# PKU-EPIC/PartManip

Hardware: AMD Instinct MI355X
Metric: PPO env-steps/sec (whole node), 4096 envs x 1024-pt clouds (higher is better)
Workload: dtype f32

## Files before the change

include/partmanip_hip.h:

```cpp
#ifndef PARTMANIP_HIP_H
#define PARTMANIP_HIP_H

#include <stddef.h>
#include <stdint.h>

#ifdef __cplusplus
extern "C" {
#endif

#define PM_OK 0
#define PM_EINVAL (-1)
#define PM_EWORKSPACE (-2)
#define PM_EALIGN (-3)
#define PM_EUNSUPPORTED (-4)

#define PM_ACT_NONE 0
#define PM_ACT_TANH 1
#define PM_ACT_RELU 2
#define PM_ACT_LRELU 3
#define PM_ACT_ELU 4
#define PM_ACT_SELU 5
#define PM_ACT_SIGMOID 6
#define PM_ACT_MAX 6

// ... 11 lines not shown
int pm_adv_normalize_f32(float* x, long n, float eps, void* workspace, size_t workspace_bytes, void* stream);

int pm_gather_rows_f32(const float* src, const int64_t* idx, float* dst, long n_rows, long row_elems,
                       long src_ld, long dst_ld, void* stream);

int pm_linear_fwd_f32(const float* X, long ldx, const float* W, long ldw, const float* b, float* Y, long ldy,
                      int M, int N, int K, int act, void* stream);
int pm_linear_bwd_data_f32(const float* dY, long lddy, const float* W, long ldw, const float* H, long ldh,
                           float* dX, long lddx, int M, int N, int K, int act, void* stream);
size_t pm_linear_bwd_weight_workspace_bytes(int M, int N, int K);
int pm_linear_bwd_weight_f32(const float* dY, long lddy, const float* X, long ldx, float* dW, long lddw,
                             float* db, int M, int N, int K, void* workspace, size_t workspace_bytes,
                             void* stream);

int pm_mlp_fwd_f32(const float* X, long ldx, int M, int n_layers, const int* dims, const float* const* W, const float* const* b,
                   int act, float* const* H, void* stream);
size_t pm_mlp_bwd_workspace_bytes(int M, int n_layers, const int* dims);
int pm_mlp_bwd_f32(const float* X, long ldx, int M, int n_layers, const int* dims, const float* const* W, const float* const* H,
                   int act, const float* dY, float* const* dW, float* const* db, float* dX, void* workspace,
                   size_t workspace_bytes, void* stream);

#define PM_LINEAR_GROUP_MAX 8
typedef struct pm_linear_fwd_desc {
    const float* X; long ldx; const float* W; long ldw; const float* b; float* Y; long ldy; int M, N, K, act;
} pm_linear_fwd_desc;
typedef struct pm_linear_bwd_data_desc {
    const float* dY; long lddy; const float* W; long ldw; const float* H; long ldh; float* dX; long lddx; int M, N, K, act;
} pm_linear_bwd_data_desc;
typedef struct pm_linear_bwd_weight_desc {
    const float* dY; long lddy; const float* X; long ldx; float* dW; long lddw; float* db; long slab_stride; int M, N, K;
    int dy_cols, x_cols;
    int pad_;
} pm_linear_bwd_weight_desc;
int pm_linear_fwd_group_f32(int n, const pm_linear_fwd_desc* d, void* stream);
int pm_linear_bwd_data_group_f32(int n, const pm_linear_bwd_data_desc* d, void* stream);
int pm_linear_bwd_weight_group_f32(int n, const pm_linear_bwd_weight_desc* d, int splits, void* stream);
#define PM_LINEAR_PATH_SKINNY 0
#define PM_LINEAR_PATH_REG 1
#define PM_LINEAR_PATH_DMA 2
typedef struct pm_linear_variant {
    int path;
    int tm, tn;
    int lay;
    int stages;
    int vec;
    int big;
    int grid;
    int n;
    int vecC[PM_LINEAR_GROUP_MAX];
    int splits[PM_LINEAR_GROUP_MAX];
    int kchunk[PM_LINEAR_GROUP_MAX];
} pm_linear_variant;
int pm_linear_fwd_variant_f32(const float* X, long ldx, const float* W, long ldw, const float* b, const float* Y, long ldy,
                              int M, int N, int K, int act, pm_linear_variant* out);
int pm_linear_bwd_data_variant_f32(const float* dY, long lddy, const float* W, long ldw, const float* H, long ldh,
                                   const float* dX, long lddx, int M, int N, int K, int act, pm_linear_variant* out);
int pm_linear_bwd_weight_variant_f32(const float* dY, long lddy, const float* X, long ldx, const float* dW, long lddw,
                                     const float* db, int M, int N, int K, const void* workspace, pm_linear_variant* out);
int pm_linear_fwd_group_variant_f32(int n, const pm_linear_fwd_desc* d, pm_linear_variant* out);
int pm_linear_bwd_data_group_variant_f32(int n, const pm_linear_bwd_data_desc* d, pm_linear_variant* out);
int pm_linear_bwd_weight_group_variant_f32(int n, const pm_linear_bwd_weight_desc* d, int splits, pm_linear_variant* out);
size_t pm_linear_chain_workspace_bytes(int M);
int pm_linear_fwd_chain_f32(int n, const pm_linear_fwd_desc* d, void* workspace, size_t workspace_bytes, void* stream);
int pm_linear_bwd_data_chain_f32(int n, const pm_linear_bwd_data_desc* d, void* workspace, size_t workspace_bytes, void* stream);

size_t pm_pointnet_packed_elems(void);
int pm_pointnet_pack_weights_f32(const float* W2, const float* W3, float* packed, void* stream);
int pm_pointnet_enc_fwd_f32(const float* x, long ldx, int B, int P, int C, int sub_mean, const float* W1,
                            const float* b1, const float* b2, const float* b3, const float* packed,
                            int max_mean, float* feat, long ldf, int32_t* argmax,
                            float* h2_save ,
                            int act ,
                            void* stream);
size_t pm_pointnet_packed_screen_bytes(void);
int pm_pointnet_pack_weights_screen(const float* W3, const float* b3, void* packed, void* stream);
int pm_pointnet_enc_fwd_screen_f32(const float* x, long ldx, int B, int P, int C, int sub_mean, const float* W1,
                                   const float* b1, const float* b2, const float* b3, const float* packed,
                                   const void* packed_screen, int max_mean, float* feat, long ldf, int32_t* argmax,
                                   float* h2_save, unsigned long long* counters, void* stream);
int pm_pointnet_enc_fwd_screen_sched_f32(const float* x, long ldx, int B, int P, int C, int sub_mean, const float* W1,
                                         const float* b1, const float* b2, const float* b3, const float* packed,
                                         const void* packed_screen, int max_mean, float* feat, long ldf, int32_t* argmax,
                                         float* h2_save, unsigned long long* counters, int schedule, void* stream);
size_t pm_pointnet_packed_bf3_bytes(void);
int pm_pointnet_pack_weights_bf3(const float* W2, const float* W3, void* packed, void* stream);
int pm_pointnet_enc_fwd_bf3(const float* x, long ldx, int B, int P, int C, int sub_mean, const float* W1,
                            const float* b1, const float* b2, const float* b3, const void* packed, int max_mean,
                            float* feat, long ldf, int32_t* argmax, float* h2_save ,
                            void* stream);
size_t pm_pointnet_packed_bf6_bytes(void);
int pm_pointnet_pack_weights_bf6(const float* W2, const float* W3, void* packed, void* stream);
int pm_pointnet_enc_fwd_bf6(const float* x, long ldx, int B, int P, int C, int sub_mean, const float* W1,
                            const float* b1, const float* b2, const float* b3, const void* packed, int max_mean,
                            float* feat, long ldf, int32_t* argmax, float* h2_save ,
                            void* stream);
size_t pm_pointnet_enc_bwd_workspace_bytes(int B, int P, int C);
int pm_pointnet_enc_bwd_f32(const float* x, long ldx, int B, int P, int C, int sub_mean, const float* W1,
                            const float* b1, const float* b2, const float* W3, const float* packed,
                            int max_mean, const float* dfeat, long ldf, const int32_t* argmax, float* dW1,
                            float* db1, float* dW2, float* db2, float* dW3, float* db3,
                            const float* h2_saved ,
                            int act , void* workspace, size_t workspace_bytes, void* stream);
int pm_pointnet_enc_bwd_w4_f32(const float* x, long ldx, int B, int P, int C, int sub_mean, const float* W1,
                               const float* b1, const float* b2, const float* W3, const float* packed,
                               int max_mean, const float* dfeat, long ldf, const int32_t* argmax, float* dW1,
                               float* db1, float* dW2, float* db2, float* dW3, float* db3, const float* h2_saved,
                               int act, void* workspace, size_t workspace_bytes, void* stream);
size_t pm_pointnet_packed_bwd_bf6_bytes(void);
int pm_pointnet_pack_weights_bwd_bf6(const float* W2, void* packed, void* stream);
int pm_pointnet_enc_bwd_bf6(const float* x, long ldx, int B, int P, int C, int sub_mean, const float* W1,
                            const float* b1, const float* b2, const float* W3, const float* packed,
                            const void* packed_w2_bf6, int max_mean, const float* dfeat, long ldf, const int32_t* argmax,
                            float* dW1, float* db1, float* dW2, float* db2, float* dW3, float* db3, const float* h2_saved,
                            void* workspace, size_t workspace_bytes, void* stream);

int pm_ppo_actor_loss_fwd_bwd_f32(const float* mu, long ldmu, const float* log_std, const float* actions,
                                  long lda, const float* old_logp, const float* adv, const float* old_mu,
                                  long ldom, const float* old_sigma, long ldos, int B, int A, float max_action,
                                  int act_tanh, float eps_clip, float desired_kl, const double* adv_moments,
                                  double adv_count, float* scal_out, float* dmu, long lddmu, float* dlog_std,
                                  void* workspace, size_t workspace_bytes, void* stream);
size_t pm_ppo_actor_loss_workspace_bytes(int B);
int pm_ppo_actor_head_supported(const float* H, long ldh, const float* W, long ldw, int A, int K, const float* dH, long lddh);
int pm_ppo_actor_head_f32(const float* H, long ldh, const float* W, long ldw, const float* bias, int K, int hidden_act,
                          const float* log_std, const float* actions, long lda, const float* old_logp, const float* adv,
                          const float* old_mu, long ldom, const float* old_sigma, long ldos, int B, int A, float max_action,
                          int act_tanh, float eps_clip, float desired_kl, const double* adv_moments, double adv_count,
                          float* scal_out, float* mu_out, long ldmu, float* dmu, long lddmu, float* dH, long lddh,
                          float* dlog_std, void* workspace, size_t workspace_bytes, unsigned int* counter, void* stream);
int pm_gaussian_logp_f32(const float* mu, long ldmu, const float* log_std, const float* actions, long lda,
                         int B, int A, float max_action, int act_tanh, float* logp, float* entropy,
                         void* stream);

int pm_value_loss_fwd_bwd_f32(const float* V, const float* returns, const float* old_values, int B,
                              int clipped, float eps_clip, const float* clip_mean_extern, float grad_scale,
                              float* scal_out, float* dV, long lddv, void* stream);

size_t pm_value_head_workspace_bytes(void);
int pm_value_head_supported(const float* H, long ldh, const float* W, int K, const float* dH, long lddh);
int pm_value_head_f32(const float* H, long ldh, const float* W, const float* bias, int K, int hidden_act, const float* returns,
                      const float* old_values, int B, int clipped, float eps_clip, const float* clip_mean_extern,
                      float grad_scale, float* scal_out, float* V_out, float* dV, long lddv, float* dH, long lddh,
                      void* workspace, size_t workspace_bytes, unsigned int* counter, void* stream);

int pm_mse_tanh_loss_fwd_bwd_f32(const float* stu_mu, long lds, const float* tea_mu, long ldt, int B, int A,
                                 float max_action, int act_tanh, float grad_scale, float* scal_out,
                                 float* dstu_mu, long ldd, void* stream);
int pm_action_activation_f32(const float* mu, float* out, long n, float max_action, int act_tanh, void* stream);
int pm_gaussian_logp_bwd_f32(const float* mu, long ldmu, const float* log_std, const float* actions, long lda, int B, int A,
                             float max_action, int act_tanh, const float* dlogp, const float* dent, float* dmu, long lddm,
                             float* dlog_std, void* stream);
int pm_action_activation_bwd_f32(const float* out, const float* dout, float* dmu, long n, float max_action, int act_tanh,
                                 void* stream);

size_t pm_clip_adam_workspace_bytes(long n);
typedef struct pm_clip_adam_desc {
    float* params; float* grads; float* exp_avg; float* exp_avg_sq; long n, n_clip; const float* extra; long extra_stride;
    long n_sum; int n_extra; float max_norm; double lr, b1, b2, eps; int32_t* state; const float* skip_flag;
    float* gnorm_out; void* workspace;
    float* stats_acc; const float* stats_scal; int stats_which;
    float grad_scale; float dp_kl_desired; float* dp_scal;
} pm_clip_adam_desc;
int pm_clip_adam_group_f32(int n, const pm_clip_adam_desc* d, void* stream);
int pm_grad_slab_sum_f32(float* grads, const float* extra, long extra_stride, long n_sum, int n_extra, void* stream);
int pm_clip_adam_step_f32(float* params, const float* grads, float* exp_avg, float* exp_avg_sq, long n,
                          long n_clip, float max_norm, double lr, double b1, double b2, double eps,
// ... 323 lines not shown
```

partmanip_amd/_lib.py:

```python
import ctypes as C
import os

import torch

HERE = os.path.dirname(os.path.abspath(__file__))
LIB_PATH = os.environ.get("PARTMANIP_HIP_LIB") or os.path.join(HERE, "lib", "libpartmanip_hip.so")

P, I, L, F, D, Z = C.c_void_p, C.c_int, C.c_long, C.c_float, C.c_double, C.c_size_t

SIGNATURES = {
    "pm_version": (I, []),
    "pm_gae_scan_f32": (I, [P, P, P, P, P, P, P, I, I, F, F, I, F, P]),
    "pm_moments_workspace_bytes": (Z, [L]),
    "pm_moments_f64": (I, [P, L, P, P, Z, P]),
    "pm_normalize_apply_f32": (I, [P, L, P, D, F, P]),
    "pm_gather_rows_f32": (I, [P, P, P, L, L, L, L, P]),
    "pm_linear_fwd_f32": (I, [P, L, P, L, P, P, L, I, I, I, I, P]),
    "pm_linear_bwd_data_f32": (I, [P, L, P, L, P, L, P, L, I, I, I, I, P]),
    "pm_linear_bwd_weight_workspace_bytes": (Z, [I, I, I]),
    "pm_linear_bwd_weight_f32": (I, [P, L, P, L, P, L, P, I, I, I, P, Z, P]),
    "pm_linear_fwd_group_f32": (I, [I, P, P]),
    "pm_linear_bwd_data_group_f32": (I, [I, P, P]),
    "pm_linear_chain_workspace_bytes": (C.c_size_t, [I]),
    "pm_linear_fwd_chain_f32": (I, [I, P, P, C.c_size_t, P]),
    "pm_linear_bwd_data_chain_f32": (I, [I, P, P, C.c_size_t, P]),
    "pm_linear_bwd_weight_group_f32": (I, [I, P, I, P]),
    "pm_linear_fwd_variant_f32": (I, [P, L, P, L, P, P, L, I, I, I, I, P]),
    "pm_linear_bwd_data_variant_f32": (I, [P, L, P, L, P, L, P, L, I, I, I, I, P]),
    "pm_linear_bwd_weight_variant_f32": (I, [P, L, P, L, P, L, P, I, I, I, P, P]),
    "pm_linear_fwd_group_variant_f32": (I, [I, P, P]),
    "pm_linear_bwd_data_group_variant_f32": (I, [I, P, P]),
    "pm_linear_bwd_weight_group_variant_f32": (I, [I, P, I, P]),
    "pm_clip_adam_group_f32": (I, [I, P, P]),
    "pm_grad_slab_sum_f32": (I, [P, P, L, L, I, P]),
    "pm_pointnet_packed_elems": (Z, []),
    "pm_pointnet_pack_weights_f32": (I, [P, P, P, P]),
    "pm_pointnet_enc_fwd_f32": (I, [P, L, I, I, I, I, P, P, P, P, P, I, P, L, P, P, I, P]),
    "pm_pointnet_packed_screen_bytes": (Z, []),
    "pm_pointnet_pack_weights_screen": (I, [P, P, P, P]),
    "pm_pointnet_enc_fwd_screen_f32": (I, [P, L, I, I, I, I, P, P, P, P, P, P, I, P, L, P, P, P, P]),
    "pm_pointnet_enc_fwd_screen_sched_f32": (I, [P, L, I, I, I, I, P, P, P, P, P, P, I, P, L, P, P, P, I, P]),
    "pm_pointnet_packed_bf3_bytes": (Z, []),
    "pm_pointnet_pack_weights_bf3": (I, [P, P, P, P]),
    "pm_pointnet_enc_fwd_bf3": (I, [P, L, I, I, I, I, P, P, P, P, P, I, P, L, P, P, P]),
    "pm_pointnet_packed_bf6_bytes": (Z, []),
    "pm_pointnet_pack_weights_bf6": (I, [P, P, P, P]),
    "pm_pointnet_enc_fwd_bf6": (I, [P, L, I, I, I, I, P, P, P, P, P, I, P, L, P, P, P]),
    "pm_pointnet_enc_bwd_workspace_bytes": (Z, [I, I, I]),
    "pm_pointnet_enc_bwd_f32": (I, [P, L, I, I, I, I, P, P, P, P, P, I, P, L, P, P, P, P, P, P, P, P, I, P, Z, P]),
    "pm_pointnet_enc_bwd_w4_f32": (I, [P, L, I, I, I, I, P, P, P, P, P, I, P, L, P, P, P, P, P, P, P, P, I, P, Z, P]),
    "pm_pointnet_packed_bwd_bf6_bytes": (Z, []),
    "pm_pointnet_pack_weights_bwd_bf6": (I, [P, P, P]),
    "pm_pointnet_enc_bwd_bf6": (I, [P, L, I, I, I, I, P, P, P, P, P, P, I, P, L, P, P, P, P, P, P, P, P, P, Z, P]),
    "pm_ppo_actor_loss_fwd_bwd_f32": (I, [P, L, P, P, L, P, P, P, L, P, L, I, I, F, I, F, F, P, D, P, P, L, P, P, Z, P]),
    "pm_ppo_actor_loss_workspace_bytes": (Z, [I]),
    "pm_ppo_actor_head_supported": (I, [P, L, P, L, I, I, P, L]),
    "pm_ppo_actor_head_f32": (I, [P, L, P, L, P, I, I, P, P, L, P, P, P, L, P, L, I, I, F, I, F, F, P, D, P, P, L, P, L, P, L, P, P, Z, P, P]),
    "pm_gaussian_logp_f32": (I, [P, L, P, P, L, I, I, F, I, P, P, P]),
    "pm_gaussian_logp_bwd_f32": (I, [P, L, P, P, L, I, I, F, I, P, P, P, L, P, P]),
    "pm_action_activation_bwd_f32": (I, [P, P, P, L, F, I, P]),
    "pm_value_loss_fwd_bwd_f32": (I, [P, P, P, I, I, F, P, F, P, P, L, P]),
    "pm_value_head_workspace_bytes": (Z, []),
    "pm_value_head_supported": (I, [P, L, P, I, P, L]),
    "pm_value_head_f32": (I, [P, L, P, P, I, I, P, P, I, I, F, P, F, P, P, P, L, P, L, P, Z, P, P]),
    "pm_mse_tanh_loss_fwd_bwd_f32": (I, [P, L, P, L, I, I, F, I, F, P, P, L, P]),
    "pm_action_activation_f32": (I, [P, P, L, F, I, P]),
    "pm_clip_adam_workspace_bytes": (Z, [L]),
    "pm_clip_adam_step_f32": (I, [P, P, P, P, L, L, F, D, D, D, D, P, P, P, P, Z, P]),
    "pm_ppo_accumulate_stats_f32": (I, [P, P, I, P]),
    "pm_fps_workspace_bytes": (Z, [I, I]),
    "pm_fps_f32": (I, [P, I, I, I, I, P, P, Z, P]),
    "pm_ball_query_f32": (I, [P, P, I, I, I, F, I, P, P]),
    "pm_group_points_f32": (I, [P, P, I, I, I, I, I, P, P]),
    "pm_group_points_bwd_f32": (I, [P, P, I, I, I, I, I, P, P]),
    "pm_group_concat_f32": (I, [P, P, P, P, I, I, I, I, I, I, P, P]),
    "pm_group_concat_bwd_f32": (I, [P, P, I, I, I, I, I, I, P, P]),
    "pm_maxpool_rows_f32": (I, [P, L, I, I, P, L, P, P]),
    "pm_maxpool_rows_bwd_f32": (I, [P, L, P, L, I, I, P, P, P]),
    "pm_depth_backproject_f32": (I, [P, I, I, I, I, P, F, F, F, F, P, P, P, P]),
    "pm_depth_compact_f32": (I, [P, I, I, P, P, P]),
    "pm_depth_cloud_f32": (I, [P, I, I, I, I, P, F, F, F, F, P, P, I, P, P, P, P]),
    "pm_cloud_gather_labeled_f32": (I, [P, P, I, I, P, I, P, L, I, F, P, L, P]),
    "pm_fps_varlen_f32": (I, [P, I, I, I, I, P, I, P, P, Z, P]),
    "pm_fps_varlen_workspace_bytes": (Z, [I, I]),
    "pm_tsdf_select_f32": (I, [P, I, I, F, F, P, P, P]),
    "pm_gaussian_sample_f32": (I, [P, L, P, P, I, I, F, I, P, P, P, P]),
    "pm_rms_update_workspace_bytes": (Z, [I]),
    "pm_rms_update_f32": (I, [P, L, I, I, I, P, P, P, P, Z, P]),
    "pm_rms_normalize_f32": (I, [P, L, I, I, P, P, P, L, P]),
    "pm_rms_moments_f64": (I, [P, L, I, I, P, P, Z, P]),
    "pm_rms_apply_moments_f32": (I, [P, L, I, I, P, P, P, P]),
    "pm_tsdf_sparse_gather_f32": (I, [P, P, P, I, I, I, P, P]),
    "pm_im2col3d_f32": (I, [P, I, I, I, I, I, I, I, I, L, L, L, L, L, P, I, P]),
    "pm_conv3d_c1_supported": (I, [I, I]),
    "pm_conv3d_c1_wgrad_workspace_bytes": (Z, [I]),
    "pm_conv3d_c1_fwd_f32": (I, [P, I, I, I, I, I, I, I, L, L, L, L, P, P, I, I, P, L, P, P]),
    "pm_conv3d_c1_wgrad_f32": (I, [P, L, P, I, I, I, I, I, I, I, L, L, L, L, I, P, L, P, P, P, Z, P]),
    "pm_col2im3d_f32": (I, [P, I, I, I, I, I, I, I, I, L, L, L, L, L, P, I, P, I, P]),
    "pm_tsdf_integrate_f32": (I, [P, P, P, I, I, L, L, F, F, P, P]),
    "pm_mesh_tsdf_query_f32": (I, [P, P, P, P, P, P, P, I, I, I, I, I, F, F, F, F, F, P, I, P, L, I, P]),
    "pm_mesh_tsdf_query_groups_f32": (I, [P, P, P, P, P, P, I, I, P, I, P, I, P, P, I, I, I, I, I, F, F, F, F, F, P, I, P, L, I, P]),
    "pm_mesh_sdf_bake_workspace_bytes": (Z, [I]),
    "pm_mesh_sdf_bake_f32": (I, [P, I, I, I, I, F, F, F, F, F, I, P, P, Z, P]),
    "pm_mesh_pc_query_f32": (I, [P, P, I, P, P, I, I, P, L, I, P, L, P]),
    "pm_mesh_pc_query_labeled_f32": (I, [P, P, I, P, P, I, I, P, L, I, P, L, P, P]),
    "pm_mesh_depth_render_f32": (I, [P, P, I, P, I, P, P, I, I, P, I, F, F, F, F, I, I, F, F, P, L, P]),
    "pm_mesh_frame_workspace_bytes": (Z, [I, I, I, I]),
    "pm_mesh_frame_render_f32": (I, [P, P, I, P, I, P, P, I, I, P, I, F, F, F, F, I, I, F, F, P, I, P, F, F, I, I, I, P, L, P, L, P, L, P, Z,
                                     P]),
    "pm_mesh_depth_render_groups_f32": (I, [P, P, I, P, I, I, P, I, P, I, P, P, I, I, P, I, F, F, F, F, I, I, F, F, P, L, P]),
    "pm_mesh_frame_render_groups_f32": (I, [P, P, I, P, I, I, P, I, P, I, P, P, I, I, P, I, F, F, F, F, I, I, F, F, P, I, P, F, F, I, I, I,
                                            P, L, P, L, P, L, P, Z, P]),
    "pm_body_pose_gather_f32": (I, [P, L, P, I, I, P, I, P, P, P]),
    "pm_grasp_cube_post_f32": (I, [P, P, P, I, I, I, I, I, I, I, P, P, P, P, P, F, P, P, P, I, P, L, P, L, P, P, P, P, L, P, P, P]),
    "pm_franka_control_f32": (I, [P, L, I, P, P, I, I, I, I, I, P, P, P, F, I, P, P, P, I, I, I, P, P, P, P, P, P, I, P]),
    "pm_franka_control_mobile_f32": (I, [P, L, I, P, P, I, I, I, I, I, P, P, P, F, I, I, P, P, P, P, I, I, I, P, P, P, P, P, P, I, P]),
    "pm_open_drawer_post_f32": (I, [P, L, P, L, P, I, I, I, I, I, I, I, P, P, P, I, P, P, P, P, P, P, F, P, P, I, P, L, P, P, P, P, P, L, P, P, P,
                                    P, P, P]),
    "pm_open_drawer_reset_f32": (I, [P, P, P, I, I, I, I, I, P, P, I, P, F, F, P, P, P, P, L, P, P, P, P]),
    "pm_articulation_step_f32": (I, [P, P, P, P, P, P, P, P, P, P, F, P, L, P, L, P, L, P, P, L, L, P, L, I, I, I, P, P, P]),
    "pm_articulation_objects_step_f32": (I, [P, P, I, I, I, I, I, P, P, P, P, P, P, P, P, P, P, P, P, L, P, P, P, L, P, L, P, P, P, P, F, I, P]),
    "pm_free_body_step_f32": (I, [P, L, P, P, P, I, I, P, P, P, P, P, F, F, F, F, I, P]),
    "pm_voxel_grid0_f32": (I, [P, L, I, I, I, I, P, P, P, P]),
    "pm_voxel_nbr27_i32": (I, [P, L, P, I, P, I, P]),
# ... 129 lines not shown
```

partmanip_amd/build.py:

```python
import os
import subprocess
import sys

HERE = os.path.dirname(os.path.abspath(__file__))
CSRC = os.path.join(HERE, "csrc")
LIBDIR = os.path.join(HERE, "lib")
LIB = os.path.join(LIBDIR, "libpartmanip_hip.so")
SOURCES = ["gae.hip", "losses.hip", "adam.hip", "gemm_f32.hip", "gemm2_f32.hip", "pointnet_enc.hip", "pointnet_enc_bf3.hip", "pointnet_enc_bf6.hip", "pointops.hip", "sa_fused.hip", "sa_groupall.hip", "conv3d.hip", "sparse_voxel.hip", "bn_pool2d.hip", "mesh_tsdf.hip", "mesh_bake.hip", "mesh_pc.hip", "mesh_depth.hip", "mesh_frame.hip", "body_pose.hip", "task_grasp_cube.hip", "task_open_drawer.hip", "articulation.hip", "articulation_objects.hip", "free_body.hip"]
FLAGS = ["-O3", "-std=c++17", "--offload-arch=gfx950", "-fPIC", "-ffp-contract=off", "-Wall",
         "-Wno-unused-function"]


def _newer(a, b):
    return (not os.path.exists(b)) or os.path.getmtime(a) > os.path.getmtime(b)


def build(force=False, verbose=False):
    hipcc = os.environ.get("HIPCC", "/opt/rocm/bin/hipcc")
    os.makedirs(LIBDIR, exist_ok=True)
    objdir = os.path.join(LIBDIR, "obj")
    os.makedirs(objdir, exist_ok=True)
    hdrs = [os.path.join(CSRC, "common.h"), os.path.join(CSRC, "mfma_f32.h"), os.path.join(CSRC, "gemm2.h"), os.path.join(CSRC, "skinny.h"), os.path.join(CSRC, "pointnet_enc_bwd_bf6.h"), os.path.join(CSRC, "pointnet_enc_screen.h"), os.path.join(CSRC, "task_common.h"), os.path.join(CSRC, "articulation_common.h"), os.path.join(CSRC, "mesh_raster.h"),
            os.path.join(HERE, "..", "include", "partmanip_hip.h")]
    objs, rebuilt = [], False
    procs = []
    for src in SOURCES:
        s = os.path.join(CSRC, src)
        o = os.path.join(objdir, src.replace(".hip", ".o"))
        objs.append(o)
        if force or _newer(s, o) or any(_newer(h, o) for h in hdrs):
            cmd = [hipcc, "-x", "hip", "-c", s, "-o", o] + FLAGS
            if verbose:
                print(" ".join(cmd))
            procs.append((src, subprocess.Popen(cmd, stdout=subprocess.PIPE, stderr=subprocess.STDOUT)))
            rebuilt = True
    for src, p in procs:
        out, _ = p.communicate()
        if p.returncode != 0:
            sys.stderr.write(out.decode())
            raise RuntimeError(f"hipcc failed on {src}")
        if verbose and out:
            print(out.decode())
    if rebuilt or not os.path.exists(LIB):
        cmd = [hipcc, "-shared", "-fPIC", "--offload-arch=gfx950", "-o", LIB] + objs
        subprocess.run(cmd, check=True)
    return LIB


if __name__ == "__main__":
    print(build(force="--force" in sys.argv, verbose=True))
```

partmanip_amd/csrc/pointnet_enc_screen.h:

```cpp
#pragma once

typedef _Float16 ps_f16x8 __attribute__((ext_vector_type(8)));

#define PS_LDP (PN_C2 + 8)
#define PS_CAP 256
#define PS_NW 8
#define PS_P3 (16 * 16 * 64 * 8)
#define PS_OFF_P3 0
#define PS_OFF_W3 (2 * PS_P3)
#define PS_OFF_EPS (PS_OFF_W3 + PN_C3 * PN_C2 * 4)
#define PS_OFF_INV (PS_OFF_EPS + PN_C3 * 4)
#define PS_PACKED_BYTES (PS_OFF_INV + PN_C3 * 4)
#ifndef PS_ABLATE
#define PS_ABLATE 0
#endif
#ifndef PS_SCHED_DEFAULT
#define PS_SCHED_DEFAULT 0
#endif

extern "C" size_t pm_pointnet_packed_screen_bytes(void) { return PS_PACKED_BYTES; }

__device__ __forceinline__ unsigned ps_cvt_pk(float a, float b) {
    unsigned r;
    asm("v_cvt_pk_f16_f32 %0, %1, %2" : "=v"(r) : "v"(a), "v"(b));
    return r;
}

__global__ __launch_bounds__(PN_C2) void ps_pack_kernel(const float* __restrict__ W3, const float* __restrict__ b3,
                                                         unsigned char* __restrict__ packed) {
    __shared__ double Ls[PN_C2], Rs[PN_C2], Ss[PN_C2];
    __shared__ float Ms[PN_C2];
    const int c = blockIdx.x, k = threadIdx.x;
    const float w = W3[c * PN_C2 + k];
    const float aw = fabsf(w);
    Ls[k] = (double)aw;
    Ms[k] = aw < INFINITY ? aw : 0.f;
    __syncthreads();
    for (int o = PN_C2 / 2; o > 0; o >>= 1) {
        if (k < o) {
            Ls[k] += Ls[k + o];
            Ms[k] = fmaxf(Ms[k], Ms[k + o]);
        }
        __syncthreads();
    }
    int ex = -200;
    if (Ms[0] > 0.f) frexpf(Ms[0], &ex);
    const int s = min(15 - ex, 126);
    const float ws = ldexpf(w, s);
    const _Float16 w16 = (_Float16)ws;
    const float wf = (float)w16, d = fabsf(ws - wf);
    Rs[k] = (double)(fabsf(wf) < 0x1p-14f ? fmaxf(fabsf(ws), d) : d);
    Ss[k] = (double)fabsf(wf);
    __syncthreads();
    for (int o = PN_C2 / 2; o > 0; o >>= 1) {
        if (k < o) {
            Rs[k] += Rs[k + o];
            Ss[k] += Ss[k + o];
        }
        __syncthreads();
    }
    const int nb = c >> 5, li = c & 31, step = k >> 4, lq = (k >> 3) & 1, e = k & 7;
    ((_Float16*)(packed + PS_OFF_P3))[(((nb * 16 + step) * 64) + lq * 32 + li) * 8 + e] = w16;
    ((float*)(packed + PS_OFF_W3))[c * PN_C2 + k] = w;
    if (k == 0) {
        const double ed = ((Rs[0] + 0x1p-12 * Ss[0]) * ldexp(1.0, -s) + 1024.0 * 0x1p-24 * (Ls[0] + fabs((double)b3[c]))) * (1.0 + 0x1p-10) + 0x1p-116;
        float ef = (float)ed;
        if ((double)ef < ed) ef = __uint_as_float(__float_as_uint(ef) + 1);
        ((float*)(packed + PS_OFF_EPS))[c] = ef;
        ((float*)(packed + PS_OFF_INV))[c] = ldexpf(1.f, -s);
    }
}

extern "C" int pm_pointnet_pack_weights_screen(const float* W3, const float* b3, void* packed, void* stream) {
    PM_REQUIRE(W3 && b3 && packed);
    if (((uintptr_t)packed & 15) != 0) return PM_EALIGN;
    hipLaunchKernelGGL(ps_pack_kernel, dim3(PN_C3), dim3(PN_C2), 0, pm_stream(stream), W3, b3, (unsigned char*)packed);
    PM_CHECK_LAUNCH();
    return PM_OK;
}

#define PS_MFMA(a, b, c) __builtin_amdgcn_mfma_f32_32x32x16_f16((a), (b), (c), 0, 0, 0)
__device__ __forceinline__ ps_f16x8 ps_h(const uint4& v) { return *(const ps_f16x8*)&v; }

__device__ __forceinline__ void ps_stream(const unsigned short* __restrict__ A, const uint4* __restrict__ B, f32x16 (&acc)[2][2]) {
    uint4 b0[2], b1[2], b2[2], b3[2], a0[2], a1[2];
#pragma unroll
    for (int nb = 0; nb < 2; ++nb) {
        b0[nb] = B[(size_t)(nb * 16 + 0) * 64];
        b1[nb] = B[(size_t)(nb * 16 + 1) * 64];
        b2[nb] = B[(size_t)(nb * 16 + 2) * 64];
    }
#pragma unroll
    for (int mb = 0; mb < 2; ++mb) a0[mb] = *(const uint4*)(A + mb * 32 * PS_LDP);
#define PS_STEP(S_, AC, AN, BC, BN, PFA, PFB)                                                  \
    {                                                                                          \
        if (PFA) {                                                                             \
            _Pragma("unroll") for (int mb = 0; mb < 2; ++mb)                                   \
                AN[mb] = *(const uint4*)(A + mb * 32 * PS_LDP + ((S_) + 1) * 16);              \
        }                                                                                      \
        if (PFB) {                                                                             \
            _Pragma("unroll") for (int nb = 0; nb < 2; ++nb)                                   \
                BN[nb] = B[(size_t)(nb * 16 + (S_) + 3) * 64];                                 \
        }                                                                                      \
// ... 89 lines not shown
    const float invr[2] = {invg[(wave * 2 + 0) * 32 + li0], invg[(wave * 2 + 1) * 32 + li0]};
    float w1r[4] = {0.f, 0.f, 0.f, 0.f}, b1r = 0.f;
    if constexpr (CT == 3 || CT == 4) layer1_row<CT>(W1, b1, w1r, b1r);

    const int ntiles = P / PN_TM;
    stage_points<PN_TM, NT>(xb, 0, C, sub_mean, cen, Xs);
    for (int tile = 0; tile < ntiles; ++tile) {
        int lane = lane0;
        asm volatile("" : "+v"(lane));
        const int li = lane & 31, lh = lane >> 5;
        PS_STAMP(0);
        __syncthreads();
        float xnext = 0.f;
        if (tile + 1 < ntiles) xnext = ps_point_load(xb, tile + 1, C, tid);
        if (!(PS_ABLATE & 1)) {
            if constexpr (CT == 3 || CT == 4) layer1_tile<CT, PN_TM, NT, true>(Xs, w1r, b1r, H);
            else layer1_tile<CT, PN_TM, NT, true>(Xs, W1, b1, C, H);
        }
        PS_STAMP(1);
        __syncthreads();
        {
            f32x16 acc2[2][1];
            zero_acc<2, 1>(acc2);
            if (PS_ABLATE & 2) {
#pragma unroll
                for (int mb = 0; mb < 2; ++mb)
#pragma unroll
                    for (int r = 0; r < 16; ++r)
                        acc2[mb][0][r] = H[(mb * 32 + (r & 3) + 8 * (r >> 2) + 4 * lh) * PN_LD1 + ((wave * 32 + li) & 127)];
            } else {
                layer2_mfma<2, 1>(H, P2v, wave, lane, acc2);
            }
            PS_STAMP(2);
            __syncthreads();
            PS_STAMP(3);
            const int col = wave * 32 + li;
            const float b2c = b2r;
            float ts = 0.f;
            const bool planes = !(PS_ABLATE & 8) || tile == 0;
            const bool odd = (lane & 1) != 0;
            unsigned* Hh2 = (unsigned*)(Hh + (odd ? PS_LDP : 0) + (col & ~1));
#pragma unroll
            for (int mb = 0; mb < 2; ++mb)
#pragma unroll
                for (int r = 0; r < 16; r += 2) {
                    const float z0 = acc2[mb][0][r] + b2c, z1 = acc2[mb][0][r + 1] + b2c;
                    f32x2 v2;
                    if (PS_ABLATE & 4) {
                        v2.x = z0;
                        v2.y = z1;
                    } else {
                        v2 = pm_tanh2(z0, z1);
                    }
                    const int row0 = mb * 32 + (r & 3) + 8 * (r >> 2) + 4 * lh;
                    H[row0 * PN_LD2 + col] = v2.x;
                    H[(row0 + 1) * PN_LD2 + col] = v2.y;
                    ts += v2.x;
                    ts += v2.y;
                    const float own = odd ? v2.y : v2.x, send = odd ? v2.x : v2.y;
                    const float recv = __int_as_float(__builtin_amdgcn_update_dpp(0, __float_as_int(send), 0xB1, 0xf, 0xf, false));
                    const float a = odd ? recv : own, c = odd ? own : recv;
                    if (planes) Hh2[row0 * (PS_LDP / 2)] = ps_cvt_pk(a, c);
                }
            ts += __shfl_xor(ts, 32, 64);
            csum += (double)ts;
            if (tile + 1 < ntiles) ps_point_store(xnext, sub_mean, cen, tid, Xs);
        }
        PS_STAMP(4);
        __syncthreads();
        PS_STAMP(5);

        const bool copy = h2_save && !(PS_ABLATE & 128), late = ps_late_wave<SCHED>(wave);
        float* h2dst = copy ? h2_save + ((long)b * P + (long)tile * PN_TM) * PN_C2 : nullptr;
        if (copy && late) ps_copy_h2<NT>(H, h2dst, tid);

        f32x16 acc[2][2];
        if (PS_ABLATE & 16) {
#pragma unroll
            for (int nb = 0; nb < 2; ++nb)
#pragma unroll
                for (int mb = 0; mb < 2; ++mb)
#pragma unroll
                    for (int r = 0; r < 16; ++r)
                        acc[mb][nb][r] = b3r[nb] + H[(mb * 32 + (r & 3) + 8 * (r >> 2) + 4 * lh) * PN_LD2 + ((wave * 64 + nb * 32 + li) & 255)];
        } else {
            zero_acc<2, 2>(acc);
            ps_stream(Hh + li * PS_LDP + lh * 8, S3 + (size_t)(wave * 2 * 16) * 64 + lane, acc);
        }
        PS_STAMP(6);

        unsigned msk[2];
        float tmax[2];
#if (PS_ABLATE & 32) && defined(__HIP_DEVICE_COMPILE__)
#pragma unroll
        for (int nb = 0; nb < 2; ++nb) {
#pragma unroll
            for (int mb = 0; mb < 2; ++mb) asm volatile("" ::"v"(acc[mb][nb]));
            msk[nb] = 0;
            tmax[nb] = 0.f;
        }
#else
#pragma unroll
        for (int nb = 0; nb < 2; ++nb) {
            float m = -INFINITY;
            const float iv = invr[nb], b3c = b3r[nb];
#pragma unroll
            for (int mb = 0; mb < 2; ++mb)
#pragma unroll
                for (int r = 0; r < 16; ++r) {
                    if (!(PS_ABLATE & 16)) acc[mb][nb][r] = fmaf(acc[mb][nb][r], iv, b3c);
                    m = fmaxf(m, acc[mb][nb][r]);
                }
            m = fmaxf(m, __shfl_xor(m, 32, 64));
            const float e = epsr[nb];
            const float vm = __shfl(vmax, nb * 32 + li, 64);
            const float thr = m - 2.f * e;
            unsigned k = 0;
#pragma unroll
            for (int mb = 0; mb < 2; ++mb)
#pragma unroll
                for (int r = 0; r < 16; ++r) {
                    const float z = acc[mb][nb][r];
                    const bool s = !(z < thr) && !(z + e <= vm);
                    k |= (s ? 1u : 0u) << (mb * 16 + r);
                }
            msk[nb] = k;
            tmax[nb] = m;
        }
#endif
        const int n = __popc(msk[0]) + __popc(msk[1]);
        int incl = n;
#pragma unroll
        for (int o = 1; o < 64; o <<= 1) {
            const int t = __shfl_up(incl, o, 64);
            if (lane >= o) incl += t;
        }
        const int total = __builtin_amdgcn_readlane(incl, 63);
        PS_STAMP(7);

        if (PS_ABLATE & 64) {
            vmax = fmaxf(vmax, lh ? tmax[1] : tmax[0]);
            if (counters && lane == 0) atomicAdd(counters + 0, (unsigned long long)total);
        } else if (total <= PS_CAP) {
            int off = incl - n;
#pragma unroll
            for (int nb = 0; nb < 2; ++nb) {
                unsigned m = msk[nb];
                while (m) {
                    const int bit = __ffs(m) - 1;
                    m &= m - 1;
                    const int row = (bit >> 4) * 32 + (bit & 3) + 8 * ((bit & 15) >> 2) + 4 * lh;
                    skey[wave][off++] = (row << 6) | (nb * 32 + li);
                }
            }
            __builtin_amdgcn_wave_barrier();
            const int j = lane & 7, g = lane >> 3;
            for (int e0 = 0; e0 < total; e0 += 8) {
                const int e = e0 + g;
                const int key = (e < total) ? skey[wave][e] : 0;
                const int row = key >> 6, cl = key & 63;
                const float* hp = H + row * PN_LD2 + 4 * j;
                const float* wp = W3r + (size_t)(wave * 64 + cl) * PN_C2 + 4 * j;
                float s = 0.f;
#pragma unroll
                for (int i = 0; i < 8; ++i) {
                    const float4 w = *(const float4*)(wp + 32 * i);
                    const float4 h = *(const float4*)(hp + 32 * i);
                    s = fmaf(w.x, h.x, s);
                    s = fmaf(w.y, h.y, s);
                    s = fmaf(w.z, h.z, s);
                    s = fmaf(w.w, h.w, s);
                }
                s += __shfl_xor(s, 4, 64);
                s += __shfl_xor(s, 2, 64);
                s += __shfl_xor(s, 1, 64);
                s += b3[wave * 64 + cl];
#pragma unroll
                for (int gg = 0; gg < 8; ++gg)
                    if (e0 + gg < total) {
                        const int kk = __builtin_amdgcn_readlane(key, gg * 8);
                        const float v = __int_as_float(__builtin_amdgcn_readlane(__float_as_int(s), gg * 8));
                        if ((kk & 63) == lane) {
                            const int p = tile * PN_TM + (kk >> 6);
                            if (!(fabsf(v) < INFINITY)) pois += v;
                            if (v > vmax || (v == vmax && p < imax)) {
                                vmax = v;
                                imax = p;
                            }
                        }
                    }
            }
            if (counters) {
                const unsigned long long h0 = __ballot(msk[0] != 0), h1 = __ballot(msk[1] != 0);
                if (lane == 0) {
                    atomicAdd(counters + 0, (unsigned long long)total);
                    atomicAdd(counters + 2, (unsigned long long)(__popc((unsigned)(h0 | (h0 >> 32))) + __popc((unsigned)(h1 | (h1 >> 32)))));
                }
            }
        } else {
#pragma unroll
            for (int nb = 0; nb < 2; ++nb) {
                const float b3c = b3r[nb];
#pragma unroll
                for (int r = 0; r < 16; ++r) acc[0][nb][r] = acc[1][nb][r] = b3c;
            }
            mfma_stream<2, 2, 32>(H + li * PN_LD2 + lh * 128, PN_LD2, P3v + (size_t)(wave * 2) * 32 * 64 + lane, acc);
#pragma unroll
            for (int nb = 0; nb < 2; ++nb) {
                float bv = -INFINITY, ps = 0.f;
                int bp = 0;
#pragma unroll
                for (int mb = 0; mb < 2; ++mb)
#pragma unroll
                    for (int r = 0; r < 16; ++r) {
                        const float v = acc[mb][nb][r];
                        if (!(fabsf(v) < INFINITY)) ps += v;
                        if (v > bv) {
                            bv = v;
                            bp = tile * PN_TM + mb * 32 + (r & 3) + 8 * (r >> 2) + 4 * lh;
                        }
                    }
                const float ov = __shfl_xor(bv, 32, 64), os = __shfl_xor(ps, 32, 64);
                const int op = __shfl_xor(bp, 32, 64);
                if (ov > bv || (ov == bv && op < bp)) {
                    bv = ov;
                    bp = op;
                }
                if (lh == nb) {
                    pois += ps + os;
                    if (bv > vmax || (bv == vmax && bp < imax)) {
                        vmax = bv;
                        imax = bp;
                    }
                }
            }
            if (counters && lane == 0) atomicAdd(counters + 1, 1ull);
        }
        PS_STAMP(8);
        if (copy && !late) ps_copy_h2<NT>(H, h2dst, tid);
        PS_STAMP(9);
    }
    if ((lane0 >> 5) == 0) cs[wave * 32 + lane0] = csum;
    __syncthreads();
    const int ch = tid;
    float v = vmax;
    if (pois != pois) v = pois;
    feat[(long)b * ldf + ch] = v;
    argmax[(long)b * PN_C3 + ch] = imax;
    if (max_mean) {
        const float* wr = W3r + (size_t)ch * PN_C2;
        double s = 0.0;
#pragma unroll 4
        for (int k = 0; k < PN_C2; k += 4) {
            const float4 w = *(const float4*)(wr + k);
            s = fma((double)w.x, cs[k], s);
            s = fma((double)w.y, cs[k + 1], s);
            s = fma((double)w.z, cs[k + 2], s);
            s = fma((double)w.w, cs[k + 3], s);
        }
        float mv = (float)(s / (double)P + (double)b3[ch]);
        if (pois != pois) mv = pois;
        feat[(long)b * ldf + PN_C3 + ch] = mv;
    }
}

extern "C" int pm_pointnet_enc_fwd_screen_sched_f32(const float* x, long ldx, int B, int P, int C, int sub_mean, const float* W1,
                                                    const float* b1, const float* b2, const float* b3, const float* packed,
                                                    const void* packed_screen, int max_mean, float* feat, long ldf,
                                                    int32_t* argmax, float* h2_save, unsigned long long* counters, int schedule,
                                                    void* stream) {
    PM_REQUIRE(x && W1 && b1 && b2 && b3 && packed && packed_screen && feat && argmax);
    PM_REQUIRE(schedule == 0 || schedule == 1);
    if (h2_save && ((uintptr_t)h2_save & 15) != 0) return PM_EALIGN;
    PM_REQUIRE(B > 0 && P > 0 && P % PN_TM == 0 && C >= 1 && C <= PN_MAXC && ldx >= (long)P * C);
    PM_REQUIRE(ldf >= PN_C3 * (max_mean ? 2 : 1));
    PM_REQUIRE(!sub_mean || C >= 3);
// ... 27 lines not shown
```

Before: 35970.

## Screen candidates in raw accumulator space with per-column thresholds and ballot compaction

```diff
diff --git a/include/partmanip_hip.h b/include/partmanip_hip.h
--- a/include/partmanip_hip.h
+++ b/include/partmanip_hip.h
@@ -117,6 +117,8 @@
                                          const float* b1, const float* b2, const float* b3, const float* packed,
                                          const void* packed_screen, int max_mean, float* feat, long ldf, int32_t* argmax,
                                          float* h2_save, unsigned long long* counters, int schedule, void* stream);
+int pm_pointnet_screen_select_thresholds(const float* mt, const float* eps, const float* b3, const float* inv, const float* vmax,
+                                         long n, float* T);
 size_t pm_pointnet_packed_bf3_bytes(void);
 int pm_pointnet_pack_weights_bf3(const float* W2, const float* W3, void* packed, void* stream);
 int pm_pointnet_enc_fwd_bf3(const float* x, long ldx, int B, int P, int C, int sub_mean, const float* W1,
diff --git a/partmanip_amd/_lib.py b/partmanip_amd/_lib.py
--- a/partmanip_amd/_lib.py
+++ b/partmanip_amd/_lib.py
@@ -40,6 +40,7 @@
     "pm_pointnet_pack_weights_screen": (I, [P, P, P, P]),
     "pm_pointnet_enc_fwd_screen_f32": (I, [P, L, I, I, I, I, P, P, P, P, P, P, I, P, L, P, P, P, P]),
     "pm_pointnet_enc_fwd_screen_sched_f32": (I, [P, L, I, I, I, I, P, P, P, P, P, P, I, P, L, P, P, P, I, P]),
+    "pm_pointnet_screen_select_thresholds": (I, [P, P, P, P, P, L, P]),
     "pm_pointnet_packed_bf3_bytes": (Z, []),
     "pm_pointnet_pack_weights_bf3": (I, [P, P, P, P]),
     "pm_pointnet_enc_fwd_bf3": (I, [P, L, I, I, I, I, P, P, P, P, P, I, P, L, P, P, P]),
diff --git a/partmanip_amd/build.py b/partmanip_amd/build.py
--- a/partmanip_amd/build.py
+++ b/partmanip_amd/build.py
@@ -20,7 +20,7 @@
     os.makedirs(LIBDIR, exist_ok=True)
     objdir = os.path.join(LIBDIR, "obj")
     os.makedirs(objdir, exist_ok=True)
-    hdrs = [os.path.join(CSRC, "common.h"), os.path.join(CSRC, "mfma_f32.h"), os.path.join(CSRC, "gemm2.h"), os.path.join(CSRC, "skinny.h"), os.path.join(CSRC, "pointnet_enc_bwd_bf6.h"), os.path.join(CSRC, "pointnet_enc_screen.h"), os.path.join(CSRC, "task_common.h"), os.path.join(CSRC, "articulation_common.h"), os.path.join(CSRC, "mesh_raster.h"),
+    hdrs = [os.path.join(CSRC, "common.h"), os.path.join(CSRC, "mfma_f32.h"), os.path.join(CSRC, "gemm2.h"), os.path.join(CSRC, "skinny.h"), os.path.join(CSRC, "pointnet_enc_bwd_bf6.h"), os.path.join(CSRC, "pointnet_enc_screen.h"), os.path.join(CSRC, "pointnet_enc_screen_select.h"), os.path.join(CSRC, "task_common.h"), os.path.join(CSRC, "articulation_common.h"), os.path.join(CSRC, "mesh_raster.h"),
             os.path.join(HERE, "..", "include", "partmanip_hip.h")]
     objs, rebuilt = [], False
     procs = []
diff --git a/partmanip_amd/csrc/pointnet_enc_screen.h b/partmanip_amd/csrc/pointnet_enc_screen.h
--- a/partmanip_amd/csrc/pointnet_enc_screen.h
+++ b/partmanip_amd/csrc/pointnet_enc_screen.h
@@ -1,4 +1,5 @@
 #pragma once
+#include "pointnet_enc_screen_select.h"
 
 typedef _Float16 ps_f16x8 __attribute__((ext_vector_type(8)));
 
@@ -19,6 +20,13 @@
 #endif
 
 extern "C" size_t pm_pointnet_packed_screen_bytes(void) { return PS_PACKED_BYTES; }
+
+extern "C" int pm_pointnet_screen_select_thresholds(const float* mt, const float* eps, const float* b3, const float* inv,
+                                                    const float* vmax, long n, float* T) {
+    PM_REQUIRE(mt && eps && b3 && inv && vmax && T && n >= 0);
+    for (long i = 0; i < n; ++i) T[i] = ps_select_threshold(mt[i], eps[i], b3[i], inv[i], vmax[i]);
+    return PM_OK;
+}
 
 __device__ __forceinline__ unsigned ps_cvt_pk(float a, float b) {
     unsigned r;
@@ -274,77 +282,74 @@
                 for (int mb = 0; mb < 2; ++mb)
 #pragma unroll
                     for (int r = 0; r < 16; ++r)
-                        acc[mb][nb][r] = b3r[nb] + H[(mb * 32 + (r & 3) + 8 * (r >> 2) + 4 * lh) * PN_LD2 + ((wave * 64 + nb * 32 + li) & 255)];
+                        acc[mb][nb][r] = ps_pow2_inverse(invr[nb]) * H[(mb * 32 + (r & 3) + 8 * (r >> 2) + 4 * lh) * PN_LD2 + ((wave * 64 + nb * 32 + li) & 255)];
         } else {
             zero_acc<2, 2>(acc);
             ps_stream(Hh + li * PS_LDP + lh * 8, S3 + (size_t)(wave * 2 * 16) * 64 + lane, acc);
         }
         PS_STAMP(6);
 
-        unsigned msk[2];
-        float tmax[2];
+        float T[2], tmax[2];
+        int total = 0;
+        unsigned long long hit[2] = {0ull, 0ull};
 #if (PS_ABLATE & 32) && defined(__HIP_DEVICE_COMPILE__)
 #pragma unroll
         for (int nb = 0; nb < 2; ++nb) {
 #pragma unroll
             for (int mb = 0; mb < 2; ++mb) asm volatile("" ::"v"(acc[mb][nb]));
-            msk[nb] = 0;
-            tmax[nb] = 0.f;
+            T[nb] = tmax[nb] = 0.f;
         }
 #else
 #pragma unroll
         for (int nb = 0; nb < 2; ++nb) {
             float m = -INFINITY;
-            const float iv = invr[nb], b3c = b3r[nb];
 #pragma unroll
             for (int mb = 0; mb < 2; ++mb)
 #pragma unroll
+                for (int r = 0; r < 16; ++r) m = fmaxf(m, acc[mb][nb][r]);
+            m = fmaxf(m, __shfl_xor(m, 32, 64));
+            const float mt = fmaf(m, invr[nb], b3r[nb]);
+            const float vm = __shfl(vmax, nb * 32 + li, 64);
+            T[nb] = ps_select_threshold(mt, epsr[nb], b3r[nb], invr[nb], vm);
+            tmax[nb] = mt;
+        }
+        int* const sk = skey[wave];
+#pragma unroll
+        for (int nb = 0; nb < 2; ++nb) {
+            const int kbase = (4 * lh) << 6 | (nb * 32 + li);
+#pragma unroll
+            for (int mb = 0; mb < 2; ++mb) {
+                bool sv[16];
+                unsigned long long mk[16];
+#pragma unroll
                 for (int r = 0; r < 16; ++r) {
-                    if (!(PS_ABLATE & 16)) acc[mb][nb][r] = fmaf(acc[mb][nb][r], iv, b3c);
-                    m = fmaxf(m, acc[mb][nb][r]);
-                }
-            m = fmaxf(m, __shfl_xor(m, 32, 64));
-            const float e = epsr[nb];
-            const float vm = __shfl(vmax, nb * 32 + li, 64);
-            const float thr = m - 2.f * e;
-            unsigned k = 0;
-#pragma unroll
-            for (int mb = 0; mb < 2; ++mb)
+                    sv[r] = !(acc[mb][nb][r] < T[nb]);
+                    mk[r] = __ballot(sv[r]);
+                }
+                __builtin_amdgcn_sched_barrier(0);
 #pragma unroll
                 for (int r = 0; r < 16; ++r) {
-                    const float z = acc[mb][nb][r];
-                    const bool s = !(z < thr) && !(z + e <= vm);
-                    k |= (s ? 1u : 0u) << (mb * 16 + r);
-                }
-            msk[nb] = k;
-            tmax[nb] = m;
+                    const bool s = sv[r];
+                    const unsigned long long mask = mk[r];
+                    if (__builtin_expect(mask != 0, 0)) {
+                        const int cnt = __popcll(mask);
+                        if (s && total + cnt <= PS_CAP) {
+                            const int pos = __builtin_amdgcn_mbcnt_hi((unsigned)(mask >> 32), __builtin_amdgcn_mbcnt_lo((unsigned)mask, total));
+                            sk[pos] = kbase + ((mb * 32 + (r & 3) + 8 * (r >> 2)) << 6);
+                        }
+                        total += cnt;
+                        hit[nb] |= mask;
+                    }
+                }
+            }
         }
 #endif
-        const int n = __popc(msk[0]) + __popc(msk[1]);
-        int incl = n;
-#pragma unroll
-        for (int o = 1; o < 64; o <<= 1) {
-            const int t = __shfl_up(incl, o, 64);
-            if (lane >= o) incl += t;
-        }
-        const int total = __builtin_amdgcn_readlane(incl, 63);
         PS_STAMP(7);
 
         if (PS_ABLATE & 64) {
             vmax = fmaxf(vmax, lh ? tmax[1] : tmax[0]);
             if (counters && lane == 0) atomicAdd(counters + 0, (unsigned long long)total);
         } else if (total <= PS_CAP) {
-            int off = incl - n;
-#pragma unroll
-            for (int nb = 0; nb < 2; ++nb) {
-                unsigned m = msk[nb];
-                while (m) {
-                    const int bit = __ffs(m) - 1;
-                    m &= m - 1;
-                    const int row = (bit >> 4) * 32 + (bit & 3) + 8 * ((bit & 15) >> 2) + 4 * lh;
-                    skey[wave][off++] = (row << 6) | (nb * 32 + li);
-                }
-            }
             __builtin_amdgcn_wave_barrier();
             const int j = lane & 7, g = lane >> 3;
             for (int e0 = 0; e0 < total; e0 += 8) {
@@ -383,7 +388,7 @@
                     }
             }
             if (counters) {
-                const unsigned long long h0 = __ballot(msk[0] != 0), h1 = __ballot(msk[1] != 0);
+                const unsigned long long h0 = hit[0], h1 = hit[1];
                 if (lane == 0) {
                     atomicAdd(counters + 0, (unsigned long long)total);
                     atomicAdd(counters + 2, (unsigned long long)(__popc((unsigned)(h0 | (h0 >> 32))) + __popc((unsigned)(h1 | (h1 >> 32)))));
diff --git a/partmanip_amd/csrc/pointnet_enc_screen_select.h b/partmanip_amd/csrc/pointnet_enc_screen_select.h
--- /dev/null
+++ b/partmanip_amd/csrc/pointnet_enc_screen_select.h
@@ -0,0 +1,20 @@
+#pragma once
+#include <math.h>
+
+#if defined(__HIPCC__)
+#define PS_HD __host__ __device__
+#else
+#define PS_HD
+#endif
+
+PS_HD inline float ps_below(float x) { return fmaf(-fabsf(x), 0x1p-23f, x) - 0x1p-149f; }
+
+PS_HD inline float ps_pow2_inverse(float inv) { return __builtin_bit_cast(float, 0x7F000000u - __builtin_bit_cast(unsigned, inv)); }
+
+PS_HD inline float ps_select_threshold(float mt, float eps, float b3, float inv, float vmax) {
+    const float sc = ps_pow2_inverse(inv);
+    const float thr1 = mt - 2.f * eps;
+    const float t1 = ps_below(ps_below(ps_below(thr1) - b3) * sc);
+    const float t2 = ps_below(ps_below(ps_below(vmax - eps) - b3) * sc);
+    return (t1 != t1 || t2 != t2) ? NAN : fmaxf(t1, t2);
+}
```

Result: no change. 36030, median of 4 (+0.2%).
